# sumitsk/algp

Hardware: AMD Instinct MI355X
Metric: GP-fit+MI-score throughput (N train x M candidates) (higher is better)
Workload: dtype f64

## Files before the change

algp_amd/csrc/api_candidates.hip:

```cpp
#include "api_impl.h"

using namespace algp;

namespace algp {


template <typename T>
int Impl<T>::set_candidates(algp_ctx* c, const int64_t* idx, int64_t M, int prior_noise, const void* extra) {
    if (c->pool_is_cov && !prior_noise)
        return fail(c, ALGP_ERR_BAD_ARG, "an explicit pool covariance carries sigma_n^2 on its diagonal: prior_includes_noise must be 1");
    const int64_t Mpad = round_up(std::max<int64_t>(M, 1), NB);
    c->M = M;
    c->Mpad = Mpad;
    c->prior_noise = prior_noise;
    c->cand_idx.assign(idx, idx + M);
    c->cand_pos.assign(c->n_pool, -1);
    for (int64_t j = 0; j < M; ++j) c->cand_pos[idx[j]] = j;
    ALGP_TRY(ensure(c, c->Cidx, sizeof(int64_t) * Mpad));
    if (M > 0) ALGP_HIP(hipMemcpyAsync(c->Cidx.p, idx, sizeof(int64_t) * M, hipMemcpyHostToDevice, c->stream));
    if (extra) {
        ALGP_TRY(ensure(c, c->cextra, sizeof(T) * Mpad));
        ALGP_HIP(hipMemcpyAsync(c->cextra.p, extra, sizeof(T) * M, hipMemcpyHostToDevice, c->stream));
    } else {
        release(c, c->cextra);
    }
    ALGP_TRY(sync(c));
    c->solved = false;
    return ALGP_OK;
}

template <typename T>
void Impl<T>::plan_route(algp_ctx* c, int incremental, bool allow_fold, typename Impl<T>::SolvePlan& pl) {
    const bool tail_on = env_switch("ALGP_TAIL_COLS", true), solve_dag_on = env_switch("ALGP_SOLVE_DAG", true),
               stats_on = env_switch("ALGP_ROW_STATS", true), fold_on = allow_fold && env_switch("ALGP_FOLD", true);
    const int64_t N = c->N, Npad = c->Npad, M = c->M, Mpad = c->Mpad;
    pl.carried_sums = incremental && c->uw_rows == N && c->uvec.p && c->wvec.p;
    int64_t keep = 0;
    if (incremental && c->Vt.p && c->vt_hyp_stamp == c->hyp_stamp && c->vt_prior_noise == c->prior_noise &&
        !c->vt_has_extra && !c->cextra.p && c->vt_cand_idx == c->cand_idx) {
        const int64_t lim = std::min<int64_t>((int64_t)c->vt_fact_idx.size(), N);
        int64_t p0 = 0;
        while (p0 < lim && c->vt_fact_idx[p0] == c->fact_idx[p0] && c->vt_fact_var[p0] == c->fact_var[p0]) ++p0;
        keep = p0 / NB * NB;
        if (tail_on && p0 >= 2048 && Mpad >= 2048 && c->cur == c->stream) {
            const bool exact = N > p0 && N - p0 <= 64;
            const int64_t k16 = exact ? p0 : p0 / 16 * 16, c1 = exact ? N : round_up(N, 16);
            int n = 0;
            bool ok = c1 > k16;
            if (exact) {
                pl.seg_c0[0] = p0;
                pl.seg_w[0] = (int)(N - p0);
                pl.seg_window = true;
                n = 1;
            }
            if (ok && !exact && c1 - k16 <= 64 && k16 / NB != (c1 - 1) / NB && k16 + NB <= Npad) {
                pl.seg_c0[0] = k16;
                pl.seg_w[0] = (int)(c1 - k16);
                pl.seg_window = true;
                n = 1;
            }
            for (int64_t a = k16; a < c1 && ok && !pl.seg_window;) {
                const int64_t b = std::min<int64_t>(c1, (a / NB + 1) * NB);
                if (b - a > 64 || n == 2) { ok = false; break; }
                pl.seg_c0[n] = a;
                pl.seg_w[n] = (int)(b - a);
                ++n;
                a = b;
            }
            if (ok && n > 0) {
                pl.nseg = n;
                keep = k16;
            }
        }
    }
    std::vector<int>& kind = pl.kind;
    kind.assign(Mpad, -1);
    if (c->prior_noise)
        for (int64_t j = 0; j < M; ++j) kind[j] = (int)c->pos_in_train[c->cand_idx[j]];
    std::vector<int64_t>& became_unit = pl.became_unit;
    became_unit.clear();
    if (keep > 0) {
        for (int64_t j = 0; j < M && keep > 0; ++j) {
            const int was = c->vt_kind[j], now = kind[j];
            if (was == now) continue;
            if (was < 0 && now >= keep) became_unit.push_back(j);
            else if (!(was >= keep && now >= keep)) keep = 0;
        }
        if (keep == 0) became_unit.clear();
    }
    if (keep == 0) { pl.nseg = 0; pl.seg_window = false; }
    pl.keep = keep;
    if (pl.nseg > 0) { pl.route = SolveRoute::Segments; return; }
    if (fold_on && M > 0 && panel_fits(Npad, Mpad)) pl.route = SolveRoute::Folded;
    else if (solve_dag_on && keep == 0 && Mpad / NB > 32 && panel_fits(Npad, Mpad) && c->cur == c->stream) pl.route = SolveRoute::TaskList;
    else pl.route = SolveRoute::Sweep;
    const int64_t r = N % NB, N1 = Npad - NB;
    const bool narrow = r > 0 && r <= 64 && N1 >= 2048 && Mpad >= 2048 && tail_on &&
                        (pl.route != SolveRoute::Sweep || (keep == 0 && c->cur == c->stream && Mpad / NB > SWEEP_PUSH_TILES));
    if (narrow) {
        pl.narrow_r = (int)r;
        pl.short_rows = pl.route == SolveRoute::Sweep ? Mpad : M < Mpad ? Mpad - NB : Mpad;
    }
    pl.row_stats = pl.route == SolveRoute::Sweep && stats_on && keep == 0 && !pl.carried_sums;
    pl.sweep_end = pl.narrow_r ? Npad - NB : Npad;
    pl.rhs_fused = pl.route == SolveRoute::Sweep && keep == 0 && M > 0 && env_switch("ALGP_RHS_FUSED", true) &&
                   trsm_sched_wanted(c, Mpad, pl.sweep_end, keep) && rhs_gen_supported(c->hyp.DP, c->pool_is_cov);
}

template <typename T>
int Impl<T>::rhs_window(algp_ctx* c, int64_t c0, int64_t w, void* out, int64_t ldo) {
    const int64_t live = std::max<int64_t>(0, std::min<int64_t>(c->N - c0, w));
    KmatSrc s = make_src(c);
    return kmat_launch<T>(c, s, (const int64_t*)c->Cidx.p, c->M, c->Mpad, (const int64_t*)c->Aidx.p + c0, live, w, nullptr, 0,
                          c->prior_noise ? (const int*)c->ckind.p : nullptr, 0, (T*)out, ldo, 0, c0);
}

template <typename T>
int Impl<T>::solve_prepare(algp_ctx* c, int incremental, typename Impl<T>::SolvePlan& pl) {
    const int64_t N = c->N, Npad = c->Npad, M = c->M, Mpad = c->Mpad, keep = pl.keep;
    const int64_t ldv = Npad + MAX_APPEND;
    c->solved = false;
    c->vr.drop();
    if (!c->Vt.p || c->ldv_cap < ldv || (keep == 0 && !incremental && c->ldv_cap != ldv) ||
        c->Vt.cap < sizeof(T) * Mpad * c->ldv_cap) {
        const int64_t newcap = incremental ? round_up(ldv + ldv / 8, NB) : ldv;
        DevBuf nv;
        ALGP_TRY(ensure(c, nv, sizeof(T) * Mpad * newcap));
        if (keep > 0) {
            hipError_t e = hipMemcpy2DAsync(nv.p, sizeof(T) * newcap, c->Vt.p, sizeof(T) * c->ldv_cap, sizeof(T) * keep,
                                            Mpad, hipMemcpyDeviceToDevice, c->stream);
            if (e != hipSuccess) { release(c, nv); return fail(c, ALGP_ERR_HIP, hipGetErrorString(e)); }
            hipStreamSynchronize(c->stream);
        }
        release(c, c->Vt);
        c->Vt = nv;
        c->ldv_cap = newcap;
    }
    const int64_t ldc = c->ldv_cap;
    c->ldv = ldc;
    ALGP_TRY(ensure(c, c->dstat, sizeof(T) * Mpad));
    ALGP_TRY(ensure(c, c->mu, sizeof(T) * Mpad));
    ALGP_TRY(ensure(c, c->tvec, sizeof(T) * 2 * Mpad));
    ALGP_TRY(ensure(c, c->alive, Mpad));
    ALGP_TRY(ensure(c, c->scores, sizeof(double) * Mpad));
    ALGP_TRY(ensure(c, c->lrow, sizeof(T) * ldc));
    ALGP_TRY(ensure(c, c->prevrows, sizeof(T) * MAX_APPEND * ldc));
    {
        ALGP_TRY(ensure(c, c->ckind, sizeof(int) * Mpad));
        ALGP_HIP(hipMemcpyAsync(c->ckind.p, pl.kind.data(), sizeof(int) * Mpad, hipMemcpyHostToDevice, c->stream));
        if (!pl.became_unit.empty() && keep > 0) {
            const size_t nb = pl.became_unit.size();
            ALGP_TRY(ensure(c, c->auxIdx, sizeof(int64_t) * nb));
            ALGP_HIP(hipMemcpyAsync(c->auxIdx.p, pl.became_unit.data(), sizeof(int64_t) * nb, hipMemcpyHostToDevice, c->stream));
            ALGP_TRY(zero_listed_rows_launch<T>(c, p(c->Vt), ldc, (const int64_t*)c->auxIdx.p, (int64_t)nb, keep));
        }
        ALGP_TRY(sync(c));
    }
    KmatSrc s = make_src(c);
    if (pl.rhs_fused) {
        const int DP = c->hyp.DP;
        ALGP_TRY(ensure(c, c->rhs_rx, sizeof(T) * (size_t)Mpad * DP));
        ALGP_TRY(ensure(c, c->rhs_cx, sizeof(T) * (size_t)Npad * DP));
        ALGP_TRY(ensure(c, c->rhs_rk, sizeof(int) * (size_t)Mpad));
        ALGP_TRY(rhs_gather_launch<T>(c, (const T*)c->Xs.p, DP, (const int64_t*)c->Cidx.p, M, Mpad,
                                      c->prior_noise ? (const int*)c->ckind.p : nullptr, (const int64_t*)c->Aidx.p, N, Npad,
                                      p(c->rhs_rx), p(c->rhs_cx), (int*)c->rhs_rk.p));
        pl.gen.rx = c->rhs_rx.p;
        pl.gen.cx = c->rhs_cx.p;
        pl.gen.rk = (const int*)c->rhs_rk.p;
        pl.gen.ncols = N;
        pl.gen.DP = DP;
        pl.gen.kernel = s.kernel;
        pl.gen.outputscale = s.outputscale;
        pl.gen.window = &Impl<T>::rhs_window;
        return rhs_window(c, pl.sweep_end, ldv - pl.sweep_end, p(c->Vt) + pl.sweep_end, ldc);
    }
    return kmat_launch<T>(c, s, (const int64_t*)c->Cidx.p, M, Mpad, (const int64_t*)c->Aidx.p + keep, N - keep,
                          ldv - keep, nullptr, 0, c->prior_noise ? (const int*)c->ckind.p : nullptr, 0,
                          p(c->Vt) + keep, ldc, 0, keep);
}


template <typename T>
int Impl<T>::solve_run(algp_ctx* c, typename Impl<T>::SolvePlan& pl) {
    const int64_t Npad = c->Npad, Mpad = c->Mpad, ldc = c->ldv, keep = pl.keep;
    prof_span_begin(c, ALGP_PROF_TRSM, (double)(Npad - keep) * (double)(Npad + keep) * (double)Mpad,
                    sizeof(T) * (double)Mpad * (double)Npad);
    int trc = ALGP_OK;
    if (pl.route == SolveRoute::Segments && pl.seg_window) {
        const int64_t w0 = std::min<int64_t>(pl.seg_c0[0], Npad - NB), o = pl.seg_c0[0] - w0;
        trc = ensure(c, c->tailE, sizeof(T) * NB * NB);
        if (trc == ALGP_OK) trc = trinv_diag_launch<T>(c, p(c->L) + w0 * c->Lld + w0, c->Lld, p(c->tailE));
        if (trc == ALGP_OK)
            trc = tail_cols_launch<T>(c, ALGP_PROF_TAIL_COLS, p(c->Vt), Mpad, ldc, p(c->L), c->Lld, Npad, (const T*)nullptr,
                                      pl.seg_c0[0], pl.seg_w[0], p(c->tailE) + o * NB + o);
    } else if (pl.route == SolveRoute::Segments) {
        for (int q = 0; q < pl.nseg && trc == ALGP_OK; ++q)
            trc = tail_cols_launch<T>(c, ALGP_PROF_TAIL_COLS, p(c->Vt), Mpad, ldc, p(c->L), c->Lld, Npad,
                                      p(c->invD) + (pl.seg_c0[q] / NB) * NB * NB, pl.seg_c0[q], pl.seg_w[q]);
    } else if (pl.route == SolveRoute::TaskList) {
        trc = solve_dag_panel<T>(c, p(c->L), Npad, c->Lld, p(c->invD), (int*)((double*)c->scal.p + SC_STALL), p(c->Vt), ldc, Mpad, 1,
                                 (int)(pl.short_rows / NB));
    } else if (pl.route == SolveRoute::Sweep) {
        T* stat = nullptr;
        if (pl.row_stats && ensure(c, c->rowstat, sizeof(T) * 2 * (size_t)(Npad / NB) * (size_t)Mpad) == ALGP_OK)
            stat = p(c->rowstat);
        trc = trsm_blocked<T>(c, ALGP_PROF_GEMM_TRSM, p(c->Vt), Mpad, ldc, p(c->L), pl.sweep_end, c->Lld, p(c->invD),
                              keep, p(c->z), stat, Mpad, &pl.rowstat_done, pl.rhs_fused ? &pl.gen : nullptr);
    } else {
        trc = fail(c, ALGP_ERR_STATE, "internal: the folded route is solved by the factorisation's launch (fit_and_solve)");
    }
    if (trc == ALGP_OK) trc = solve_narrow_tile(c, pl);
    prof_span_end(c);
    return trc;
}


template <typename T>
int Impl<T>::solve_narrow_tile(algp_ctx* c, const typename Impl<T>::SolvePlan& pl) {
    if (pl.narrow_r == 0) return ALGP_OK;
    const int64_t Mpad = c->Mpad, ldc = c->ldv, N1 = c->Npad - NB;
    ALGP_TRY(tail_cols_launch<T>(c, ALGP_PROF_TAIL_COLS, p(c->Vt), pl.short_rows, ldc, p(c->L), c->Lld, c->Npad,
                                 p(c->invD) + (N1 / NB) * NB * NB, N1, (int)round_up(pl.narrow_r, 16)));
    if (!pl.rowstat_done) return ALGP_OK;
    T* stat = p(c->rowstat);
    return rows_reduce_launch<T>(c, p(c->Vt) + N1, Mpad, ldc, NB, p(c->z) + N1, stat + 2 * (N1 / NB) * Mpad,
                                 stat + (2 * (N1 / NB) + 1) * Mpad);
}


template <typename T>
int Impl<T>::solve_finish(algp_ctx* c, int incremental, const unsigned char* alive_host, const typename Impl<T>::SolvePlan& pl) {
    const int64_t N = c->N, Npad = c->Npad, M = c->M, Mpad = c->Mpad, ldc = c->ldv, keep = pl.keep;
    T* ss = p(c->tvec);
    T* dot = ss + Mpad;
    if (pl.carried_sums) {
        const size_t need = sizeof(T) * 6 * (size_t)Mpad;
        bool ok = keep > 0 && c->acc3.p && c->acc3.cap >= need && c->acc_M == M && c->acc_cols > 0 &&
                  c->acc_cols <= keep && c->acc_cols <= c->uw_stable;
        if (!ok) {
            ALGP_TRY(ensure(c, c->acc3, need));
            ALGP_HIP(hipMemsetAsync(c->acc3.p, 0, sizeof(T) * 3 * (size_t)Mpad, c->stream));
            c->acc_cols = 0;
        }
        T* acc = p(c->acc3);
        T* tmp = acc + 3 * Mpad;
        if (!pl.became_unit.empty()) {
            const size_t nb = pl.became_unit.size();
            ALGP_TRY(ensure(c, c->auxIdx, sizeof(int64_t) * nb));
            ALGP_HIP(hipMemcpyAsync(c->auxIdx.p, pl.became_unit.data(), sizeof(int64_t) * nb, hipMemcpyHostToDevice, c->stream));
            ALGP_TRY(zero_rows3_launch<T>(c, acc, Mpad, (const int64_t*)c->auxIdx.p, (int64_t)nb));
        }
        const int64_t fin = N / NB * NB;
        if (fin > c->acc_cols)
            ALGP_TRY(rows_reduce3_launch<T>(c, p(c->Vt), M, ldc, c->acc_cols, fin, p(c->uvec), p(c->wvec), acc, Mpad, 1));
        ALGP_TRY(rows_reduce3_launch<T>(c, p(c->Vt), M, ldc, fin, Npad, p(c->uvec), p(c->wvec), tmp, Mpad, 0));
        ALGP_TRY(combine3_launch<T>(c, M, acc, tmp, Mpad, (T)c->ybar, ss, dot));
        c->acc_cols = fin;
        c->acc_M = M;
        c->uw_stable = N;
    } else {
        c->acc_cols = 0;
        if (pl.rowstat_done) ALGP_TRY(rowstat_combine_launch<T>(c, p(c->rowstat), Mpad, (int)(Npad / NB), M, ss, dot));
        else ALGP_TRY(rows_reduce_launch<T>(c, p(c->Vt), M, ldc, Npad, p(c->z), ss, dot));
    }
    const T prior = (T)(c->hyp.outputscale + (c->prior_noise ? c->hyp.noise : 0.0));
    ALGP_TRY(cand_finalize_launch<T>(c, M, (const int*)c->ckind.p, (const int64_t*)c->Cidx.p,
                                     c->pool_is_cov ? (const T*)c->Cp.p : nullptr, c->n_pool, prior,
                                     c->cextra.p ? (const T*)c->cextra.p : nullptr, ss, dot, (T)c->ybar, p(c->dstat),
                                     p(c->mu), (unsigned char*)c->alive.p));
    if (alive_host) ALGP_HIP(hipMemcpyAsync(c->alive.p, alive_host, M, hipMemcpyHostToDevice, c->stream));
    ALGP_TRY(sync_checked(c, "solve_candidates"));
    c->ncols = Npad;
    c->picks.clear();
    c->mi.valid = false;
    c->vr.drop();
    ALGP_TRY(reset_lazy(c));
    c->solved = true;
    c->vt_fact_idx = c->fact_idx;
    c->vt_fact_var = c->fact_var;
    c->vt_cand_idx = c->cand_idx;
    c->vt_kind.assign(pl.kind.begin(), pl.kind.begin() + M);
    c->vt_hyp_stamp = c->hyp_stamp;
    c->vt_prior_noise = c->prior_noise;
    c->vt_has_extra = c->cextra.p != nullptr;
    c->kept_cols_last = keep;
    return ALGP_OK;
}


template <typename T>
int Impl<T>::solve_candidates(algp_ctx* c, int incremental, const unsigned char* alive_host) {
    if (!c->factored || c->train_dirty) return fail(c, ALGP_ERR_STATE, "solve_candidates: call algp_factorize first");
    SolvePlan pl;
    plan_route(c, incremental, false, pl);
    ALGP_TRY(solve_prepare(c, incremental, pl));
    ALGP_TRY(solve_run(c, pl));
    return solve_finish(c, incremental, alive_host, pl);
}


template <typename T>
int Impl<T>::fit_and_solve(algp_ctx* c) {
    SolvePlan pl;
    plan_route(c, 0, true, pl);
    if (pl.route != SolveRoute::Folded) {
        ALGP_TRY(factorize(c, 0));
        ALGP_TRY(solve_prepare(c, 0, pl));
        ALGP_TRY(solve_run(c, pl));
        return solve_finish(c, 0, nullptr, pl);
    }
    c->factored = false;
    ALGP_TRY(solve_prepare(c, 0, pl));
    Panel pn{p(c->Vt), c->ldv, c->Mpad, 1};
    if (c->M < c->Mpad) {
        pn.z_row = c->M;
        ALGP_HIP(hipMemcpyAsync(p(c->Vt) + c->M * c->ldv, c->y0.p, sizeof(T) * c->Npad, hipMemcpyDeviceToDevice, c->stream));
    }
    pn.short_rows = pl.short_rows;
    ALGP_TRY(factorize(c, 0, &pn));
    ALGP_TRY(solve_narrow_tile(c, pl));
    return solve_finish(c, 0, nullptr, pl);
}


template <typename T>
int Impl<T>::get_posterior(algp_ctx* c, void* mu, void* var) {
    if (!c->solved) return fail(c, ALGP_ERR_STATE, "get_posterior: call algp_solve_candidates first");
    ALGP_TRY(flush_lazy(c));
    if (mu) ALGP_HIP(hipMemcpyAsync(mu, c->mu.p, sizeof(T) * c->M, hipMemcpyDeviceToHost, c->stream));
    if (var) ALGP_HIP(hipMemcpyAsync(var, c->dstat.p, sizeof(T) * c->M, hipMemcpyDeviceToHost, c->stream));
    return sync(c);
}


template <typename T>
int Impl<T>::get_posterior_cov(algp_ctx* c, void* cov_out, double* mi_out) {
    if (!c->solved) return fail(c, ALGP_ERR_STATE, "get_posterior_cov: call algp_solve_candidates first");
    if (c->pool_is_cov) return fail(c, ALGP_ERR_BAD_ARG, "get_posterior_cov needs a coordinate pool");
    const int64_t M = c->M, Mpad = c->Mpad;
    if (c->prior_noise)
        for (int64_t j = 0; j < M; ++j)
            if (c->vt_kind[j] >= 0)
                return fail(c, ALGP_ERR_STATE,
                            "get_posterior_cov: candidate " + std::to_string(j) + " (pool index " + std::to_string(c->cand_idx[j]) +
                                ") is a train site and was solved as a unit row (prior_includes_noise = 1): set the "
                                "candidates with prior_includes_noise = 0");
    if (!c->picks.empty())
        return fail(c, ALGP_ERR_STATE, "get_posterior_cov: " + std::to_string(c->picks.size()) +
                                           " pick(s) were committed since the candidate solve, which the covariance would "
                                           "not include: solve the candidates again");
    c->last_jitter = 0.0;
    if (M == 0) {
        if (mi_out) *mi_out = 0.0;
        return ALGP_OK;
    }
    ALGP_TRY(ensure(c, c->auxA, sizeof(T) * Mpad * Mpad));
    ALGP_TRY(ensure(c, c->auxW, sizeof(T) * Mpad * Mpad));
    ALGP_TRY(ensure(c, c->auxInv, sizeof(T) * Mpad * NB));
    KmatSrc s = make_src(c);
    const T* extra = c->cextra.p ? (const T*)c->cextra.p : nullptr;
    c->last_jitter = 0.0;
    const double eps = sizeof(T) == 8 ? 2.220446049250313e-16 : 1.1920928955078125e-07;
    for (int attempt = 0;; ++attempt) {
        const double jitter = attempt == 0 ? 0.0 : 64.0 * eps * c->hyp.outputscale * pow(100.0, attempt - 1);
        ALGP_TRY(kmat_launch<T>(c, s, (const int64_t*)c->Cidx.p, M, Mpad, (const int64_t*)c->Cidx.p, M, Mpad, extra, 0,
                                nullptr, 1, p(c->auxA), Mpad));
        ALGP_TRY(gemm_nt_launch<T>(c, ALGP_PROF_GEMM_OTHER, Mpad, Mpad, c->Npad, (T)-1, p(c->Vt), c->ldv, p(c->Vt),
                                   c->ldv, (T)1, p(c->auxA), Mpad, p(c->auxW), Mpad, 0));
        if (attempt == 0 && cov_out)
            ALGP_HIP(hipMemcpy2DAsync(cov_out, sizeof(T) * M, c->auxW.p, sizeof(T) * Mpad, sizeof(T) * M, M,
                                      hipMemcpyDeviceToHost, c->stream));
        ALGP_TRY(sync(c));
        if (!mi_out) break;
        if (jitter > 0.0) {
            ALGP_TRY(add_diag_launch<T>(c, p(c->auxA), M, Mpad, (T)jitter));
            ALGP_TRY(add_diag_launch<T>(c, p(c->auxW), M, Mpad, (T)jitter));
        }
        double ld_xx = 0, ld_cov = 0;
        int rc = factor_resident(c, p(c->auxA), M, Mpad, p(c->auxInv), SC_AUXLOGDET, SC_AUXINFO, &ld_xx);
        if (rc == ALGP_OK) rc = factor_resident(c, p(c->auxW), M, Mpad, p(c->auxInv), SC_AUXLOGDET, SC_AUXINFO, &ld_cov);
        if (rc == ALGP_OK) {
            *mi_out = 0.5 * (ld_xx - ld_cov);
            c->last_jitter = jitter;
            break;
        }
        if (rc != ALGP_ERR_NOT_PD || attempt >= 5) return rc;
        c->err.clear();
    }
    return ALGP_OK;
}


template <typename T>
int Impl<T>::posterior_mean(algp_ctx* c, const int64_t* idx, int64_t M, void* mu_out) {
    if (!c->factored || c->train_dirty) return fail(c, ALGP_ERR_STATE, "posterior_mean: call algp_factorize first");
    if (c->pool_is_cov) return fail(c, ALGP_ERR_BAD_ARG, "posterior_mean needs a coordinate pool");
    if (M == 0) return ALGP_OK;
    ALGP_TRY(ensure(c, c->auxIdx, sizeof(int64_t) * M));
    ALGP_TRY(ensure(c, c->auxD, sizeof(T) * M));
    ALGP_HIP(hipMemcpyAsync(c->auxIdx.p, idx, sizeof(int64_t) * M, hipMemcpyHostToDevice, c->stream));
    ALGP_TRY(need_alpha(c));
    ALGP_TRY(kgemv_launch<T>(c, M, (const int64_t*)c->auxIdx.p, make_src(c), c->N, (const int64_t*)c->Aidx.p,
                             (const T*)c->alpha.p, (T)c->ybar, p(c->auxD)));
    ALGP_HIP(hipMemcpyAsync(mu_out, c->auxD.p, sizeof(T) * M, hipMemcpyDeviceToHost, c->stream));
    const int rc = sync_checked(c, "posterior_mean");
    if (rc != ALGP_OK) c->alpha_valid = false;
    return rc;
}

template struct Impl<float>;
template struct Impl<double>;

}

extern "C" {

int algp_set_candidates(algp_ctx* c, const int64_t* idx, int64_t M, int prior_noise, const void* extra) {
    CHECK_CTX(c);
    if (c->n_pool <= 0) return fail(c, ALGP_ERR_STATE, "set_candidates: set a pool first");
    if (M < 0 || (M > 0 && !idx)) return fail(c, ALGP_ERR_BAD_ARG, "set_candidates: bad arguments");
    for (int64_t i = 0; i < M; ++i)
        if (idx[i] < 0 || idx[i] >= c->n_pool) return fail(c, ALGP_ERR_BAD_ARG, "set_candidates: index outside the pool");
    FINISH(c, DISPATCH(c, set_candidates(c, idx, M, prior_noise, extra)));
}

int algp_fit_and_solve(algp_ctx* c) {
    CHECK_CTX(c);
    NEED_HYPERS(c);
    if (c->n_pool <= 0) return fail(c, ALGP_ERR_STATE, "fit_and_solve: set a pool first");
    if (!c->y0.p || (int64_t)c->pos_in_train.size() != c->n_pool)
        return fail(c, ALGP_ERR_STATE, "fit_and_solve: call algp_set_train first");
    if ((int64_t)c->cand_pos.size() != c->n_pool) return fail(c, ALGP_ERR_STATE, "fit_and_solve: call algp_set_candidates first");
    FINISH(c, DISPATCH(c, fit_and_solve(c)));
}

int algp_solve_candidates(algp_ctx* c) { CHECK_CTX(c); FINISH(c, DISPATCH(c, solve_candidates(c, 0, nullptr))); }

int algp_solve_candidates_update(algp_ctx* c, const uint8_t* alive, int64_t* kept_cols) {
    CHECK_CTX(c);
    int rc = DISPATCH(c, solve_candidates(c, 1, alive));
    if (kept_cols) *kept_cols = rc == ALGP_OK ? c->kept_cols_last : 0;
    if (c->prof_on) prof_collect(c);
    return rc;
}

int algp_set_candidate_alive(algp_ctx* c, const uint8_t* alive) {
    CHECK_CTX(c);
    if (!c->solved || !alive) return fail(c, ALGP_ERR_STATE, "set_candidate_alive: solve the candidates first");
    if (hipMemcpyAsync(c->alive.p, alive, c->M, hipMemcpyHostToDevice, c->stream) != hipSuccess)
        return fail(c, ALGP_ERR_HIP, "set_candidate_alive: copy failed");
    c->bounds_valid = false;
    return sync(c);
}

int algp_get_posterior(algp_ctx* c, void* mu, void* var) { CHECK_CTX(c); FINISH(c, DISPATCH(c, get_posterior(c, mu, var))); }

int algp_get_posterior_cov(algp_ctx* c, void* cov, double* mi) { CHECK_CTX(c); FINISH(c, DISPATCH(c, get_posterior_cov(c, cov, mi))); }
// ... 11 lines not shown
```

algp_amd/csrc/api_impl.h:

```cpp
#pragma once
#include <limits.h>
#include <math.h>
#include <string.h>

#include <algorithm>
#include <stdlib.h>

#include "common.h"
#include "vecops.h"

namespace algp {

void release(algp_ctx* c, DevBuf& b);
void release(algp_ctx* c, MiState& mi);
void release(algp_ctx* c, VrState& vr);
hipEvent_t sync_event_api(algp_ctx* c, size_t i);
KmatSrc make_src(algp_ctx* c);
int sync(algp_ctx* c);
int sync_checked(algp_ctx* c, const char* what);
inline bool vr_over_ranks(const algp_ctx* c) { return c->vr.xrows != 0 && c->comm_nranks > 1; }

enum class SolveRoute { Segments, TaskList, Sweep, Folded };

template <typename T>
struct Impl {
    static T* p(DevBuf& b) { return (T*)b.p; }
    static int rescale_pool(algp_ctx* c);
    static int kernel_matrix(algp_ctx* c, const void* x1, int64_t n1, const void* x2, int64_t n2, const void* diag_add,
                             int add_lik, void* out);
    static int set_pool(algp_ctx* c, const void* x, int64_t n);
    static uint64_t train_sites_hash(const algp_ctx* c, const std::vector<int64_t>& idx);
    static int set_pool_cov(algp_ctx* c, const void* cov, int64_t n);
    static int set_train(algp_ctx* c, const int64_t* idx, int64_t N, const void* y, const void* var);

    struct Panel {
        T* P;
        int64_t ldp, mpad;
        int mode;
        T* inv_out = nullptr;
        bool inv_enqueued = false;
        int64_t z_row = -1;
        int64_t short_rows = 0;
    };
    static bool panel_fits(int64_t npad, int64_t mpad);
    static int factor_resident(algp_ctx* c, T* A, int64_t n, int64_t npad, T* invD, int slot_logdet, int slot_info,
                               double* logdet, int64_t ld = 0, int64_t pivot_offset = 0, Panel* panel = nullptr);
    static int reserve_factor(algp_ctx* c, int64_t npad_need, int64_t keep_rows, int64_t keep_height = 0,
                              bool headroom = false);
    static bool vt_rows_for_new_sites(algp_ctx* c, int64_t Nb, int64_t p0, std::vector<int64_t>& src_row,
                                      std::vector<int64_t>& lrow, std::vector<T>& lscale, bool& any_second);
    static int exchange_new_rows(algp_ctx* c, int64_t Nb, int64_t p0, int* placed, int st_in = 0);
    static int factorize(algp_ctx* c, int incremental, Panel* panel = nullptr);
    static int finish_factor(algp_ctx* c, int64_t keep, int64_t p0, double ld_total, T* z_src = nullptr);
    static int factorize_from(algp_ctx* c, algp_ctx* src);
    static int need_alpha(algp_ctx* c);
    static int set_candidates(algp_ctx* c, const int64_t* idx, int64_t M, int prior_noise, const void* extra);

    struct SolvePlan {
        SolveRoute route = SolveRoute::Sweep;
        int64_t keep = 0;
        std::vector<int> kind;
        std::vector<int64_t> became_unit;
        bool carried_sums = false;
        int nseg = 0;
        int64_t seg_c0[2] = {0, 0};
        int seg_w[2] = {0, 0};
        bool seg_window = false;
        int narrow_r = 0;
        int64_t short_rows = 0;
        bool row_stats = false;
        bool rowstat_done = false;
        bool rhs_fused = false;
        int64_t sweep_end = 0;
        RhsGen gen;
    };
    static int rhs_window(algp_ctx* c, int64_t c0, int64_t w, void* out, int64_t ldo);
    static constexpr int64_t SWEEP_PUSH_TILES = 320;
    static void plan_route(algp_ctx* c, int incremental, bool allow_fold, SolvePlan& pl);
    static int solve_prepare(algp_ctx* c, int incremental, SolvePlan& pl);
    static int solve_run(algp_ctx* c, SolvePlan& pl);
    static int solve_narrow_tile(algp_ctx* c, const SolvePlan& pl);
    static int solve_finish(algp_ctx* c, int incremental, const unsigned char* alive_host, const SolvePlan& pl);
    static int solve_candidates(algp_ctx* c, int incremental, const unsigned char* alive_host);
    static int fit_and_solve(algp_ctx* c);
    static int get_posterior(algp_ctx* c, void* mu, void* var);
    static int get_posterior_cov(algp_ctx* c, void* cov_out, double* mi_out);
    static int posterior_mean(algp_ctx* c, const int64_t* idx, int64_t M, void* mu_out);
    static int sample_posterior(algp_ctx* c, int S, int F, const double* omega, const double* phase, const double* weights,
                                const double* prior, const double* eps, void* out);
    static int group_posterior(algp_ctx* c, const int32_t* group, const double* weight, int64_t Q, void* mean_out, void* cov_out,
                               void* cross_out);
    static int build_set_matrix(algp_ctx* c, const int64_t* idx, int64_t m, const void* var, int64_t* mpad_out, T* dst = nullptr);
    static int set_entropy(algp_ctx* c, const int64_t* idx, int64_t m, const void* var, double* H);
    static int inverse_diag_resident(algp_ctx* c, int64_t m, int64_t mpad, void* diag_out);
    static int set_inverse_diag(algp_ctx* c, const int64_t* idx, int64_t m, const void* var, void* diag_out, double* H);
    static int upload_padded(algp_ctx* c, DevBuf& b, const void* A, int64_t rows, int64_t cols, int64_t rpad,
                             int64_t cpad);
    static int entropy_from_cov(algp_ctx* c, const void* cov, int64_t k, double* H, void* L_out, double* logdet);
    static int gemm_host(algp_ctx* c, int64_t m, int64_t n, int64_t k, double alpha, const void* A, const void* B,
                         double beta, const void* C, void* D);
    static int trsm_host(algp_ctx* c, const void* L, int64_t n, const void* B, int64_t m, void* X);
    struct MiPlan {
        std::vector<int64_t> A, Abar, all, posbar;
        std::vector<T> vA, vall;
        int64_t mb = 0, mbpad = 0, npad = 0;
        size_t rbytes = 0, cbytes = 0;
    };
    static int mi_sets(algp_ctx* c, double ss, double sm, MiPlan& pl);
    static int mi_vectors(algp_ctx* c, const MiPlan& pl, int64_t col);
    static int mi_install(algp_ctx* c, MiPlan& pl, const double* Hs, int form, double ss, double sm);
    static int mi_build(algp_ctx* c, double ss, double sm);
    static int mi_apply_pick(algp_ctx* c, int64_t q, double ss, double sm);
    static int mi_shard_plan(algp_ctx* c, double ss, double sm, MiPlan& pl);
    static int mi_shard_build(algp_ctx* c, MiPlan& pl, double* H3);
    static int mi_shard_fold(algp_ctx* c, int st);
    static int mi_shard_step(algp_ctx* c, double ss, double sm, int st, bool first_of_call);
    static int mi_scores_enqueue(algp_ctx* c, double ss, double sm, double delta, double* dst);
    static int vr_product(algp_ctx* c);
    static int vr_fold(algp_ctx* c, int64_t q);
    static int vr_scores_enqueue(algp_ctx* c, double ss, double delta, double* dst);
    static int vr_zero_picks_block(algp_ctx* c, int64_t q);
    static int vr_shard_build(algp_ctx* c, int64_t max_rows, int st = 0);
    static int vr_shard_fold(algp_ctx* c, int st);
    static int vr_shard_step(algp_ctx* c, int st, bool first_of_call);
    static int set_target_weights(algp_ctx* c, const double* w);
    static int target_variance(algp_ctx* c, double* sum);
    static int scores_enqueue(algp_ctx* c, int criterion, double static_std, double mobile_std, double* dst);
    static int scores(algp_ctx* c, int criterion, double static_std, double mobile_std, void* out, int out_is_device);
    static int argmax(algp_ctx* c, int64_t* local_pos, int64_t* pool_idx, double* value);

    struct RemoteSlots {
        int64_t* cidx;
        int* ckind;
        T *ss, *dot, *dstat, *mu;
        unsigned char* alive;
        int* fresh;
        double* score;
    };
    static RemoteSlots remote_slots(algp_ctx* c);
    static int remote_row(algp_ctx* c, int64_t pool_idx, int in_train);
    static int commit_enqueue(algp_ctx* c, int64_t pool_idx, double ss, double delta, const char* winner_payload = nullptr);
    static int commit_pick(algp_ctx* c, int64_t pool_idx, double static_std, double mobile_std);
    static int lazy_launch(algp_ctx* c, int mode, int64_t pos, double ss, double delta, const int64_t* pos_dev = nullptr);
    static int reset_lazy(algp_ctx* c);
    static int flush_lazy(algp_ctx* c);
    static int enqueue_local_best(algp_ctx* c, double ss, double delta);
    static int ensure_bounds(algp_ctx* c, int criterion, double static_std, double mobile_std, double ss, double delta);
    static int best_candidate(algp_ctx* c, int criterion, double static_std, double mobile_std, int64_t* local_pos,
                              int64_t* pool_idx, double* value);
    static int greedy_picks(algp_ctx* c, int criterion, double static_std, double mobile_std, int k, int64_t* picks_out, double* ut_out);
    static int greedy(algp_ctx* c, int criterion, double static_std, double mobile_std, int k, const int64_t* forced,
                      int64_t* picks_out, double* ut_out);
    static int score_paths_big(algp_ctx* c, const std::vector<int64_t>& cpos, const std::vector<int64_t>& lpos, int npaths, int maxlen,
                               int maxused, double mobile_std, double* dH);
    static int score_paths(algp_ctx* c, const int64_t* sites, int npaths, int maxlen, double mobile_std, double* dH);
    static int score_paths_mi(algp_ctx* c, const int64_t* sites, int npaths, int maxlen, double static_std, double mobile_std,
                              double* dMI, double* terms);
    static int score_paths_vr(algp_ctx* c, const int64_t* sites, int npaths, int maxlen, double mobile_std, int64_t max_union, double* dV);
    static int mll_grad(algp_ctx* c, double* grad_out, bool have_X = false, bool inv_enqueued = false);
    static int fit_step(algp_ctx* c, double* mll_out, double* grad_out);
    static int get_alpha(algp_ctx* c, void* out);
    static int get_factor(algp_ctx* c, void* out);
    static int selftest(algp_ctx* c, int* mism);
};

template <typename T>
int factor_blocks_batched(algp_ctx* c, T* G, int ppad, T* inv, T* L21, double* logdet, int* info, int B) {
    ALGP_TRY(potrf_diag_batched_launch<T>(c, G, (int64_t)ppad * ppad, ppad, inv, 2 * NB * NB, logdet, info, B));
    if (ppad > NB) {
        T* G21 = G + (int64_t)NB * ppad;
        T* G22 = G21 + NB;
        ALGP_TRY(gemm_nt<T>(c, {.klass = ALGP_PROF_GEMM_OTHER, .m = NB, .n = NB, .k = NB, .A = {G21, ppad, (int64_t)ppad * ppad},
                                .B = {inv, NB, 2 * NB * NB}, .D = {L21, NB, NB * NB}, .batch = B}));
        ALGP_TRY(gemm_nt<T>(c, {.klass = ALGP_PROF_GEMM_OTHER, .m = NB, .n = NB, .k = NB, .alpha = (T)-1, .beta = (T)1, .A = {L21, NB, NB * NB},
                                .B = {L21, NB, NB * NB}, .D = {G22, ppad, (int64_t)ppad * ppad}, .batch = B}));
        ALGP_TRY(potrf_diag_batched_launch<T>(c, G22, (int64_t)ppad * ppad, ppad, inv + NB * NB, 2 * NB * NB, logdet, info, B));
    }
    return ALGP_OK;
}

}

#define DISPATCH(c, call) ((c)->dtype == ALGP_F64 ? Impl<double>::call : Impl<float>::call)
#define CHECK_CTX(c) do { if (!(c)) return ALGP_ERR_BAD_ARG; (c)->err.clear(); hipSetDevice((c)->device); } while (0)
#define NEED_HYPERS(c) do { if (!(c)->hyp.set) return fail(c, ALGP_ERR_STATE, "call algp_set_hypers first"); } while (0)
#define FINISH(c, expr) do { int rc__ = (expr); if ((c)->prof_on) prof_collect(c); return rc__; } while (0)
```

algp_amd/csrc/common.h:

```cpp
#pragma once
#include <stdlib.h>
#include <hip/hip_runtime.h>
#include <stdint.h>
#include <string>
#include <type_traits>
#include <vector>
#include "../../include/algp_hip.h"

namespace algp {

constexpr int NB = 128;
constexpr int MAXD = 8;
constexpr int MAX_APPEND = 128;
constexpr double ENT_CONST = 1.4189385332046727;

inline int64_t round_up(int64_t v, int64_t m) { return (v + m - 1) / m * m; }

constexpr int SC_LOGDET = 0;
constexpr int SC_INFO = 1;
constexpr int SC_AUXLOGDET = 2;
constexpr int SC_AUXINFO = 3;
constexpr int SC_AMAXV = 4;
constexpr int SC_AMAXI = 5;
constexpr int SC_PROBE = 6;
// ... 124 lines not shown
}

__device__ __forceinline__ float kfma(float a, float b, float c) { return __builtin_fmaf(a, b, c); }
__device__ __forceinline__ double kfma(double a, double b, double c) { return __builtin_fma(a, b, c); }
template <typename T>
__device__ __forceinline__ T kval_matern_05_25(int kernel, T os, T r2, T* dk) {
#pragma clang fp contract(off)
    const bool m25 = kernel == ALGP_KERNEL_MATERN25;
    const T r = sqrt(r2);
    const T a = r * (m25 ? (T)2.2360679774997896 : (T)1);
    const T oe = os * kexp(-a);
    const T a1 = (T)1 + a;
    if (dk) *dk = m25 ? (T)1.6666666666666667 * (a1 * oe) : (r > (T)0 ? oe / r : (T)0);
    return m25 ? kfma(a * (T)0.33333333333333333, a, a1) * oe : oe;
}
__host__ __device__ inline int kernel_family(int kernel) { return kernel == ALGP_KERNEL_MATERN05 || kernel == ALGP_KERNEL_MATERN25 ? 1 : 0; }
template <typename T, int FAM = -1>
__device__ __forceinline__ T kval(int kernel, T os, T r2) {
    if (FAM != 1 && kernel == ALGP_KERNEL_RBF) return os * kexp((T)-0.5 * r2);
    if (FAM != 1 && (FAM == 0 || kernel == ALGP_KERNEL_MATERN15)) {
        const T r = sqrt(r2) * (T)1.7320508075688772;
        return os * ((T)1 + r) * kexp(-r);
    }
    return kval_matern_05_25<T>(kernel, os, r2, nullptr);
}
template <typename T, int FAM = -1>
__device__ __forceinline__ T kdk(int kernel, T os, T r2, T& dk) {
    if (FAM != 1 && kernel == ALGP_KERNEL_RBF) {
        const T kv = os * kexp((T)-0.5 * r2);
        dk = kv;
        return kv;
    }
    if (FAM != 0 && (FAM == 1 || kernel_family(kernel) == 1)) return kval_matern_05_25<T>(kernel, os, r2, &dk);
    const T a = sqrt(r2) * (T)1.7320508075688772;
    const T e = kexp(-a);
    dk = (T)3 * os * e;
    return os * ((T)1 + a) * e;
}
template <typename T, int DP, int FAM = -1>
__device__ __forceinline__ T kmat_value(int kernel, T os, const T (&xr)[DP], const T (&xc)[DP]) {
    T r2;
    if constexpr (DP == 2) {
        const T d0 = xr[0] - xc[0], d1 = xr[1] - xc[1];
        const T q1 = d1 * d1;
        r2 = kfma(d0, d0, q1);
    } else {
        r2 = (T)0;
#pragma unroll
        for (int d = 0; d < DP; ++d) {
            const T df = xr[d] - xc[d];
            r2 += df * df;
        }
    }
    return kval<T, FAM>(kernel, os, r2);
}
template <typename T, int DP>
__device__ __forceinline__ T bt_entry(int kernel, T os, const T (&xr)[DP], const T (&xc)[DP], int kind, int64_t gcol, int64_t ncols) {
    const T v = kmat_value<T, DP>(kernel, os, xr, xc);
    const T ordinary = (kind == -1 && gcol < ncols) ? v : (T)0;
    const T unit = gcol == (int64_t)kind ? (T)1 : (T)0;
    return kind >= 0 ? unit : ordinary;
}

template <typename T, typename C = T>
struct CovSrc {
    const T* Xs;
    const T* Cp;
    int64_t n_pool;
    int kernel;
    C os, noise;
};
template <int DP, bool NOISE = true, typename S, typename XA, typename XB>
__device__ __forceinline__ auto pool_cov(const S& s, int64_t pa, int64_t pb, const XA* xa, const XB* xb) {
    using C = decltype(s.os);
    if (s.Cp) return (C)s.Cp[pa * s.n_pool + pb];
    C r2 = (C)0;
#pragma unroll
    for (int d = 0; d < DP; ++d) {
        const C df = (C)xa[d] - (C)xb[d];
        r2 += df * df;
    }
    C v = kval<C>(s.kernel, s.os, r2);
    if (NOISE && pa == pb) v += s.noise;
    return v;
}
template <int DP, bool NOISE = true, typename S, typename XA>
__device__ __forceinline__ auto pool_cov(const S& s, int64_t pa, int64_t pb, const XA* xa) {
    return pool_cov<DP, NOISE>(s, pa, pb, xa, s.Xs + pb * DP);
}
template <int DP, typename S>
__device__ __forceinline__ auto pool_cov(const S& s, int64_t pa, int64_t pb) {
    return pool_cov<DP>(s, pa, pb, s.Xs + pa * DP, s.Xs + pb * DP);
}
}

struct algp_ctx {
    int device = 0;
    int dtype = ALGP_F64;
    size_t es = 8;
    hipStream_t stream = nullptr;
    hipStream_t stream2 = nullptr;
    hipStream_t stream3 = nullptr, stream4 = nullptr;
    int trsm_chunks = 3;
    bool trsm_chunks_explicit = false;
    int cu_count = 0;
    bool gemm_sched = false;
    hipStream_t cur = nullptr;
    std::vector<hipEvent_t> sync_events;
    std::string err;
    int64_t pivot = 0;
    double last_jitter = 0;
    algp::Hypers hyp;

    int64_t n_pool = 0;
    bool pool_is_cov = false;
    algp::DevBuf Xs;
    algp::DevBuf Xraw;
    algp::DevBuf Cp;
    algp::DevBuf tw;
    bool has_tw = false;
    uint64_t tw_hash = 0;
    std::vector<int64_t> pos_in_train;
    std::vector<uint64_t> site_hash;

    int64_t N = 0, Npad = 0;
    int64_t Lld = 0;
    int64_t Nfact = 0;
    std::vector<int64_t> fact_idx;
    std::vector<double> fact_var;
    std::vector<double> train_var_host;
    uint64_t fact_hyp_stamp = 0, hyp_stamp = 1;
    bool train_dirty = false;
    int64_t kept_rows_last = 0;
    std::vector<int64_t> train_idx;
    bool mean_override = false;
    double mean_value = 0;
    bool train_has_repeats = false;
    algp::DevBuf Aidx, yA, varA, y0, L, invD, z, alpha, scal;
    double ybar = 0, logdet = 0, yalpha = 0;
    bool factored = false;
    algp::DevBuf yraw, uvec, wvec;
    std::vector<double> train_y_host, fact_y;
    int64_t uw_rows = 0;
    int64_t uw_stable = 0;
    algp::DevBuf acc3;
    algp::DevBuf rowstat;
    algp::DevBuf splitk;
    algp::DevBuf ldpart;
    algp::DevBuf tailPart;
    algp::DevBuf tailE;
    algp::DevBuf gemm_part;
    algp::DevBuf inv512, inv512_scr, trsm_tmp;
    algp::DevBuf rhs_rx, rhs_cx, rhs_rk;
    std::vector<algp::DagCache> dag_cache;
    algp::DevBuf dag_state;
    algp::DevBuf trsv_ctrl;
    algp::DevBuf dag_stats;
    int64_t acc_cols = 0, acc_M = -1;
    int64_t factor_rows_from_vt = 0;
    bool alpha_valid = false;

    int64_t M = 0, Mpad = 0, ldv = 0;
    int64_t ncols = 0;
    int prior_noise = 1;
    std::vector<int64_t> cand_idx;
    std::vector<int64_t> cand_pos;
    algp::DevBuf Cidx, ckind, cextra, Vt, dstat, mu, alive, scores, lrow, tvec, amax;
    std::vector<algp::PickRec> picks;
    algp::DevBuf prevrows;
    algp::DevBuf remote;
    algp::DevBuf fresh, lazypicks;
    bool lazy_stale = false;
    bool bounds_valid = false;
    double lazy_ss = 0, lazy_delta = 0;
    bool solved = false;
    int64_t ldv_cap = 0;
    std::vector<int64_t> vt_fact_idx, vt_cand_idx;
    std::vector<double> vt_fact_var;
    std::vector<int> vt_kind;
    uint64_t vt_hyp_stamp = 0;
    int vt_prior_noise = -1;
    bool vt_has_extra = false;
    int64_t kept_cols_last = 0;

    algp::MiState mi;
    algp::VrState vr;

    void* comm = nullptr;
    algp_allgather_fn host_gather = nullptr;
    void* host_gather_user = nullptr;
    int comm_nranks = 1, comm_rank = 0;
    algp::DevBuf commbuf;
    void* comm_host = nullptr;
    size_t comm_host_cap = 0;
    std::vector<int32_t> site_owner;
    uint64_t site_owner_hash = 0;
    algp::DevBuf rowx;
    void* rowx_host = nullptr;
    size_t rowx_host_cap = 0;
    int64_t rows_from_peers = 0;
    int64_t row_exchanges = 0, row_fallbacks = 0;
    int debug_fail_next_rowx = 0;
    int pending_pick_error = 0;
    std::string pending_pick_msg;
    int64_t n_syncs = 0;
    int debug_dag_stall_ticket = -1;
    int debug_trsv_stall_block = -1;
    int debug_fail_next_pick = 0;
    int debug_fail_next_commit = 0;
    int debug_fail_next_pack = 0;
    int debug_fail_next_mi = 0;
    int debug_fail_next_vr = 0;
    double xhdr[4] = {0, 0, 0, 0};

    algp::DevBuf auxA, auxInv, auxW, auxIdx, auxVar, auxD, hostStage;
    algp::DevBuf smp;
    algp::DevBuf grp;

    bool prof_on = false;
    algp::ProfSlot prof[ALGP_PROF_COUNT];
    std::vector<algp::PendingEvent> pending;
    std::vector<hipEvent_t> event_pool;
    int64_t dev_bytes = 0;
};

namespace algp {

int fail(algp_ctx* c, int code, const std::string& msg);
int ensure(algp_ctx* c, DevBuf& b, size_t bytes);
void prof_begin(algp_ctx* c, int klass, double flops, double bytes);
void prof_end(algp_ctx* c);
bool prof_launch_events(algp_ctx* c, int klass, double flops, double bytes, hipEvent_t* a, hipEvent_t* b);
void prof_collect(algp_ctx* c);
void prof_span_begin(algp_ctx* c, int klass, double flops, double bytes);
void prof_span_end(algp_ctx* c);
void prof_span_end_on(algp_ctx* c, hipStream_t st);
void prof_span_begin2(algp_ctx* c, int klass, double flops, double bytes);
void prof_span_end2(algp_ctx* c);

inline bool env_switch(const char* name, bool dflt) {
    const char* e = getenv(name);
    return (e && *e) ? atoi(e) != 0 : dflt;
}
inline int env_int(const char* name, int dflt) {
    const char* e = getenv(name);
    return (e && *e) ? atoi(e) : dflt;
}

#define ALGP_HIP(call)                                                                          \
    do {                                                                                        \
        hipError_t e_ = (call);                                                                 \
        if (e_ != hipSuccess)                                                                   \
            return algp::fail(c, ALGP_ERR_HIP, std::string(#call) + ": " + hipGetErrorString(e_)); \
    } while (0)
#define ALGP_TRY(call)          \
    do {                        \
        int r_ = (call);        \
        if (r_ != ALGP_OK) return r_; \
    } while (0)

struct ProfScope {
    algp_ctx* c;
    ProfScope(algp_ctx* c_, int klass, double flops, double bytes) : c(c_) { prof_begin(c, klass, flops, bytes); }
    ~ProfScope() { prof_end(c); }
};

struct KmatSrc {
    const void* Xs;
    const void* Cp;
    int64_t n_pool;
    int DP;
    int kernel;
    double outputscale;
    double noise;
};
template <typename T, typename C = T>
inline CovSrc<T, C> cov_src(const KmatSrc& s) {
    return {(const T*)s.Xs, (const T*)s.Cp, s.n_pool, s.kernel, (C)s.outputscale, (C)(s.Cp ? 0.0 : s.noise)};
}
template <typename F>
inline void with_dp(int DP, F&& f) {
    if (DP == 2) f(std::integral_constant<int, 2>{});
    else if (DP == 4) f(std::integral_constant<int, 4>{});
    else f(std::integral_constant<int, 8>{});
}
#define ALGP_INSTANTIATE(f) \
    template decltype(f<double>) f<double>; \
    template decltype(f<float>) f<float>

struct RhsGen {
    const void* rx = nullptr;
    const void* cx = nullptr;
    const int* rk = nullptr;
    int64_t ncols = 0;
    int DP = 0, kernel = 0;
    double outputscale = 0;
    int (*window)(algp_ctx* c, int64_t c0, int64_t w, void* out, int64_t ldo) = nullptr;
};
template <typename T>
int rhs_gather_launch(algp_ctx* c, const T* Xs, int DP, const int64_t* ridx, int64_t rows, int64_t rows_pad, const int* unit,
                      const int64_t* cidx, int64_t cols, int64_t cols_pad, T* rx, T* cx, int* rk);
template <typename T>
int gemm_nt_launch_gen(algp_ctx* c, int klass, int64_t m, int64_t n, int64_t k, T alpha, const T* A, int64_t lda, const T* B,
                       int64_t ldb, T beta, const RhsGen& gen, int64_t col0, T* D, int64_t ldd);
bool rhs_gen_supported(int DP, bool pool_is_cov);

// ... 160 lines not shown
```

Baseline: 652,500.

## Split leftover candidate panels into the factorisation fold, sweep the rest

When the candidate tile count leaves a small remainder relative to the per-round CU capacity, the last few candidate panels are solved inside the Cholesky factorisation (folded panel), while the remaining rows go through the blocked TRSM sweep. Row counts for the sweep, RHS generation, row statistics and the narrow tail are all reduced to the sweep portion, with the split-off rows reduced separately. The goal is to avoid a poorly-occupied final round of TRSM tiles, at the cost of more routing complexity and extra work inside factorisation.

```diff
diff --git a/algp_amd/csrc/api_candidates.hip b/algp_amd/csrc/api_candidates.hip
--- a/algp_amd/csrc/api_candidates.hip
+++ b/algp_amd/csrc/api_candidates.hip
@@ -94,24 +94,37 @@
     if (fold_on && M > 0 && panel_fits(Npad, Mpad)) pl.route = SolveRoute::Folded;
     else if (solve_dag_on && keep == 0 && Mpad / NB > 32 && panel_fits(Npad, Mpad) && c->cur == c->stream) pl.route = SolveRoute::TaskList;
     else pl.route = SolveRoute::Sweep;
+    int64_t split = 0;
+    if (fold_on && pl.route != SolveRoute::TaskList && keep == 0 && M > 0 && M < Mpad && c->cur == c->stream && c->cu_count >= 2) {
+        const int forced = env_int("ALGP_SPLIT_PANELS", -1);
+        const int64_t per_round = 2 * c->cu_count / 4, left = (Mpad / NB) % per_round;
+        if (forced >= 0) split = forced;
+        else if (pl.route == SolveRoute::Sweep && left <= SPLIT_P_MAX) split = left;
+        if (!(split >= 1 && split < Mpad / NB && panel_fits(Npad, NB * split) && trsm_sched_wanted(c, Mpad - NB * split, Npad, keep)))
+            split = 0;
+        if (split) pl.route = SolveRoute::Sweep;
+    }
     const int64_t r = N % NB, N1 = Npad - NB;
     const bool narrow = r > 0 && r <= 64 && N1 >= 2048 && Mpad >= 2048 && tail_on &&
                         (pl.route != SolveRoute::Sweep || (keep == 0 && c->cur == c->stream && Mpad / NB > SWEEP_PUSH_TILES));
     if (narrow) {
         pl.narrow_r = (int)r;
-        pl.short_rows = pl.route == SolveRoute::Sweep ? Mpad : M < Mpad ? Mpad - NB : Mpad;
-    }
+        pl.short_rows = pl.route == SolveRoute::Sweep && !split ? Mpad : M < Mpad ? Mpad - NB : Mpad;
+    }
+    pl.sweep_end = pl.narrow_r ? Npad - NB : Npad;
+    pl.split_tiles = (int)split;
+    pl.sweep_rows = Mpad - NB * split;
     pl.row_stats = pl.route == SolveRoute::Sweep && stats_on && keep == 0 && !pl.carried_sums;
-    pl.sweep_end = pl.narrow_r ? Npad - NB : Npad;
     pl.rhs_fused = pl.route == SolveRoute::Sweep && keep == 0 && M > 0 && env_switch("ALGP_RHS_FUSED", true) &&
-                   trsm_sched_wanted(c, Mpad, pl.sweep_end, keep) && rhs_gen_supported(c->hyp.DP, c->pool_is_cov);
+                   trsm_sched_wanted(c, pl.sweep_rows, pl.sweep_end, keep) && rhs_gen_supported(c->hyp.DP, c->pool_is_cov);
 }
 
 template <typename T>
 int Impl<T>::rhs_window(algp_ctx* c, int64_t c0, int64_t w, void* out, int64_t ldo) {
     const int64_t live = std::max<int64_t>(0, std::min<int64_t>(c->N - c0, w));
+    const int64_t rows = c->rhs_rows;
     KmatSrc s = make_src(c);
-    return kmat_launch<T>(c, s, (const int64_t*)c->Cidx.p, c->M, c->Mpad, (const int64_t*)c->Aidx.p + c0, live, w, nullptr, 0,
+    return kmat_launch<T>(c, s, (const int64_t*)c->Cidx.p, std::min<int64_t>(c->M, rows), rows, (const int64_t*)c->Aidx.p + c0, live, w, nullptr, 0,
                           c->prior_noise ? (const int*)c->ckind.p : nullptr, 0, (T*)out, ldo, 0, c0);
 }
 
@@ -159,10 +172,12 @@
     KmatSrc s = make_src(c);
     if (pl.rhs_fused) {
         const int DP = c->hyp.DP;
-        ALGP_TRY(ensure(c, c->rhs_rx, sizeof(T) * (size_t)Mpad * DP));
+        const int64_t Ms = pl.sweep_rows;
+        c->rhs_rows = Ms;
+        ALGP_TRY(ensure(c, c->rhs_rx, sizeof(T) * (size_t)Ms * DP));
         ALGP_TRY(ensure(c, c->rhs_cx, sizeof(T) * (size_t)Npad * DP));
-        ALGP_TRY(ensure(c, c->rhs_rk, sizeof(int) * (size_t)Mpad));
-        ALGP_TRY(rhs_gather_launch<T>(c, (const T*)c->Xs.p, DP, (const int64_t*)c->Cidx.p, M, Mpad,
+        ALGP_TRY(ensure(c, c->rhs_rk, sizeof(int) * (size_t)Ms));
+        ALGP_TRY(rhs_gather_launch<T>(c, (const T*)c->Xs.p, DP, (const int64_t*)c->Cidx.p, std::min<int64_t>(M, Ms), Ms,
                                       c->prior_noise ? (const int*)c->ckind.p : nullptr, (const int64_t*)c->Aidx.p, N, Npad,
                                       p(c->rhs_rx), p(c->rhs_cx), (int*)c->rhs_rk.p));
         pl.gen.rx = c->rhs_rx.p;
@@ -173,7 +188,11 @@
         pl.gen.kernel = s.kernel;
         pl.gen.outputscale = s.outputscale;
         pl.gen.window = &Impl<T>::rhs_window;
-        return rhs_window(c, pl.sweep_end, ldv - pl.sweep_end, p(c->Vt) + pl.sweep_end, ldc);
+        ALGP_TRY(rhs_window(c, pl.sweep_end, ldv - pl.sweep_end, p(c->Vt) + pl.sweep_end, ldc));
+        if (pl.split_tiles)
+            return kmat_launch<T>(c, s, (const int64_t*)c->Cidx.p + Ms, M - Ms, Mpad - Ms, (const int64_t*)c->Aidx.p, N, ldv, nullptr, 0,
+                                  c->prior_noise ? (const int*)c->ckind.p + Ms : nullptr, 0, p(c->Vt) + Ms * ldc, ldc, 0, 0);
+        return ALGP_OK;
     }
     return kmat_launch<T>(c, s, (const int64_t*)c->Cidx.p, M, Mpad, (const int64_t*)c->Aidx.p + keep, N - keep,
                           ldv - keep, nullptr, 0, c->prior_noise ? (const int*)c->ckind.p : nullptr, 0,
@@ -184,8 +203,9 @@
 template <typename T>
 int Impl<T>::solve_run(algp_ctx* c, typename Impl<T>::SolvePlan& pl) {
     const int64_t Npad = c->Npad, Mpad = c->Mpad, ldc = c->ldv, keep = pl.keep;
-    prof_span_begin(c, ALGP_PROF_TRSM, (double)(Npad - keep) * (double)(Npad + keep) * (double)Mpad,
-                    sizeof(T) * (double)Mpad * (double)Npad);
+    const int64_t booked = pl.route == SolveRoute::Sweep ? pl.sweep_rows : Mpad;
+    prof_span_begin(c, ALGP_PROF_TRSM, (double)(Npad - keep) * (double)(Npad + keep) * (double)booked,
+                    sizeof(T) * (double)booked * (double)Npad);
     int trc = ALGP_OK;
     if (pl.route == SolveRoute::Segments && pl.seg_window) {
         const int64_t w0 = std::min<int64_t>(pl.seg_c0[0], Npad - NB), o = pl.seg_c0[0] - w0;
@@ -202,11 +222,12 @@
         trc = solve_dag_panel<T>(c, p(c->L), Npad, c->Lld, p(c->invD), (int*)((double*)c->scal.p + SC_STALL), p(c->Vt), ldc, Mpad, 1,
                                  (int)(pl.short_rows / NB));
     } else if (pl.route == SolveRoute::Sweep) {
+        const int64_t rows = pl.sweep_rows;
         T* stat = nullptr;
-        if (pl.row_stats && ensure(c, c->rowstat, sizeof(T) * 2 * (size_t)(Npad / NB) * (size_t)Mpad) == ALGP_OK)
+        if (pl.row_stats && ensure(c, c->rowstat, sizeof(T) * 2 * (size_t)(Npad / NB) * (size_t)rows) == ALGP_OK)
             stat = p(c->rowstat);
-        trc = trsm_blocked<T>(c, ALGP_PROF_GEMM_TRSM, p(c->Vt), Mpad, ldc, p(c->L), pl.sweep_end, c->Lld, p(c->invD),
-                              keep, p(c->z), stat, Mpad, &pl.rowstat_done, pl.rhs_fused ? &pl.gen : nullptr);
+        trc = trsm_blocked<T>(c, ALGP_PROF_GEMM_TRSM, p(c->Vt), rows, ldc, p(c->L), pl.sweep_end, c->Lld, p(c->invD),
+                              keep, p(c->z), stat, rows, &pl.rowstat_done, pl.rhs_fused ? &pl.gen : nullptr);
     } else {
         trc = fail(c, ALGP_ERR_STATE, "internal: the folded route is solved by the factorisation's launch (fit_and_solve)");
     }
@@ -219,13 +240,13 @@
 template <typename T>
 int Impl<T>::solve_narrow_tile(algp_ctx* c, const typename Impl<T>::SolvePlan& pl) {
     if (pl.narrow_r == 0) return ALGP_OK;
-    const int64_t Mpad = c->Mpad, ldc = c->ldv, N1 = c->Npad - NB;
+    const int64_t rows = pl.sweep_rows, ldc = c->ldv, N1 = c->Npad - NB;
     ALGP_TRY(tail_cols_launch<T>(c, ALGP_PROF_TAIL_COLS, p(c->Vt), pl.short_rows, ldc, p(c->L), c->Lld, c->Npad,
                                  p(c->invD) + (N1 / NB) * NB * NB, N1, (int)round_up(pl.narrow_r, 16)));
     if (!pl.rowstat_done) return ALGP_OK;
     T* stat = p(c->rowstat);
-    return rows_reduce_launch<T>(c, p(c->Vt) + N1, Mpad, ldc, NB, p(c->z) + N1, stat + 2 * (N1 / NB) * Mpad,
-                                 stat + (2 * (N1 / NB) + 1) * Mpad);
+    return rows_reduce_launch<T>(c, p(c->Vt) + N1, rows, ldc, NB, p(c->z) + N1, stat + 2 * (N1 / NB) * rows,
+                                 stat + (2 * (N1 / NB) + 1) * rows);
 }
 
 
@@ -261,8 +282,13 @@
         c->uw_stable = N;
     } else {
         c->acc_cols = 0;
-        if (pl.rowstat_done) ALGP_TRY(rowstat_combine_launch<T>(c, p(c->rowstat), Mpad, (int)(Npad / NB), M, ss, dot));
-        else ALGP_TRY(rows_reduce_launch<T>(c, p(c->Vt), M, ldc, Npad, p(c->z), ss, dot));
+        if (pl.rowstat_done) {
+            const int64_t Ms = pl.sweep_rows;
+            ALGP_TRY(rowstat_combine_launch<T>(c, p(c->rowstat), Ms, (int)(Npad / NB), std::min<int64_t>(M, Ms), ss, dot));
+            if (M > Ms) ALGP_TRY(rows_reduce_launch<T>(c, p(c->Vt) + Ms * ldc, M - Ms, ldc, Npad, p(c->z), ss + Ms, dot + Ms));
+        } else {
+            ALGP_TRY(rows_reduce_launch<T>(c, p(c->Vt), M, ldc, Npad, p(c->z), ss, dot));
+        }
     }
     const T prior = (T)(c->hyp.outputscale + (c->prior_noise ? c->hyp.noise : 0.0));
     ALGP_TRY(cand_finalize_launch<T>(c, M, (const int*)c->ckind.p, (const int64_t*)c->Cidx.p,
@@ -304,6 +330,18 @@
 int Impl<T>::fit_and_solve(algp_ctx* c) {
     SolvePlan pl;
     plan_route(c, 0, true, pl);
+    if (pl.split_tiles) {
+        const int64_t Ms = pl.sweep_rows;
+        c->factored = false;
+        ALGP_TRY(solve_prepare(c, 0, pl));
+        Panel pn{p(c->Vt) + Ms * c->ldv, c->ldv, c->Mpad - Ms, 1};
+        pn.z_row = c->M - Ms;
+        ALGP_HIP(hipMemcpyAsync(p(c->Vt) + c->M * c->ldv, c->y0.p, sizeof(T) * c->Npad, hipMemcpyDeviceToDevice, c->stream));
+        pn.short_rows = pl.narrow_r ? pl.short_rows - Ms : 0;
+        ALGP_TRY(factorize(c, 0, &pn));
+        ALGP_TRY(solve_run(c, pl));
+        return solve_finish(c, 0, nullptr, pl);
+    }
     if (pl.route != SolveRoute::Folded) {
         ALGP_TRY(factorize(c, 0));
         ALGP_TRY(solve_prepare(c, 0, pl));
diff --git a/algp_amd/csrc/api_impl.h b/algp_amd/csrc/api_impl.h
--- a/algp_amd/csrc/api_impl.h
+++ b/algp_amd/csrc/api_impl.h
@@ -72,8 +72,11 @@
         bool rowstat_done = false;
         bool rhs_fused = false;
         int64_t sweep_end = 0;
+        int split_tiles = 0;
+        int64_t sweep_rows = 0;
         RhsGen gen;
     };
+    static constexpr int SPLIT_P_MAX = 14;
     static int rhs_window(algp_ctx* c, int64_t c0, int64_t w, void* out, int64_t ldo);
     static constexpr int64_t SWEEP_PUSH_TILES = 320;
     static void plan_route(algp_ctx* c, int incremental, bool allow_fold, SolvePlan& pl);
diff --git a/algp_amd/csrc/common.h b/algp_amd/csrc/common.h
--- a/algp_amd/csrc/common.h
+++ b/algp_amd/csrc/common.h
@@ -300,6 +300,7 @@
     algp::DevBuf gemm_part;
     algp::DevBuf inv512, inv512_scr, trsm_tmp;
     algp::DevBuf rhs_rx, rhs_cx, rhs_rk;
+    int64_t rhs_rows = 0;
     std::vector<algp::DagCache> dag_cache;
     algp::DevBuf dag_state;
     algp::DevBuf trsv_ctrl;
```

New measurement: 659,100 (median of 6 runs). 1.01x the previous value.
